# johndpope/Emote-hack

Measured on AMD Instinct MI355X. Metric: denoised frames/s (512x512, 50-step DDPM), higher is better.
Workload: dtype bf16; 1 GPU; cfg2 (BASELINE configs[1]): 512x512 latents 64x64, 12-frame window per GPU, 50-step DDPM, CFG 7.5 (uc+c batched), ReferenceNet on (midup), motion modules res 1/2/4/8, ctx 77x768; 1 step = 1 loop iteration + 1/10 of a 10-timestep ReferenceNet pass; frames_total=12, num_inference_steps=50, latents_finite=True, hip_graphs=True, reference_group=10

## Files before the change

### emote_hack_amd/csrc/temporal.hip

```cpp
#include "common.h"

static constexpr int TA_THREADS = 256;


template <typename T>
__global__ __launch_bounds__(TA_THREADS) void temporal_attention_kernel(const T* __restrict__ qkv, int64_t ldqkv, T* __restrict__ out,
                                                                        int64_t ldo, int F, int HW, int C, int d, int hpb, int P,
                                                                        float scale, int JW, int FP) {
  constexpr int V = TT<T>::VEC;
  extern __shared__ __attribute__((aligned(16))) unsigned char smem[];
  const int CT = hpb * d;
  const int ROW = P * CT * (int)sizeof(T) + 16;
  unsigned char* Qs = smem;
  unsigned char* Ks = Qs + F * ROW;
  unsigned char* Vs = Ks + F * ROW;
  float* S = (float*)(Vs + F * ROW);

  const int tid = threadIdx.x;
  const int pix0 = blockIdx.x * P, hg = blockIdx.y, b = blockIdx.z;
  const int c0 = hg * CT;
  const int CTV = CT / V, PC = P * CTV;
  const int jl = tid % JW, rstep = TA_THREADS / JW, r0 = tid / JW;

  for (int j0 = 0; j0 < PC; j0 += JW) {
    const int j = j0 + jl;
    if (j >= PC || r0 >= rstep) break;
    const int pp = j / CTV, cv = j - pp * CTV;
    const bool pix_ok = pix0 + pp < HW;
    const T* src = qkv + ((int64_t)(b * F + r0) * HW + (pix_ok ? pix0 + pp : 0)) * ldqkv + c0 + cv * V;
    const int64_t fstep = (int64_t)rstep * HW * ldqkv;
    unsigned char* dst = smem + j * 16;
#pragma unroll 4
    for (int f = r0; f < F; f += rstep) {
      uint4 vq = make_uint4(0, 0, 0, 0), vk = vq, vv = vq;
      if (pix_ok) { vq = *(const uint4*)src; vk = *(const uint4*)(src + C); vv = *(const uint4*)(src + 2 * C); }
      *(uint4*)(dst + f * ROW) = vq;
      *(uint4*)(dst + (F + f) * ROW) = vk;
      *(uint4*)(dst + (2 * F + f) * ROW) = vv;
      src += fstep;
    }
  }
  __syncthreads();

  const int dv = d / V, NPH = P * hpb;
  {
    const int nb = (F + 2) / 3, per = nb * nb;
    for (int it = tid; it < NPH * per; it += TA_THREADS) {
      const int ph = it / per, r = it - ph * per, bq = r / nb, bk = r - bq * nb;
      const unsigned char* qp[3];
      const unsigned char* kp[3];
#pragma unroll
      for (int u = 0; u < 3; u++) {
        const int fq = bq * 3 + u < F ? bq * 3 + u : F - 1, fk = bk * 3 + u < F ? bk * 3 + u : F - 1;
        qp[u] = Qs + fq * ROW + ph * d * (int)sizeof(T);
        kp[u] = Ks + fk * ROW + ph * d * (int)sizeof(T);
      }
      float acc[3][3] = {{0.f, 0.f, 0.f}, {0.f, 0.f, 0.f}, {0.f, 0.f, 0.f}};
      for (int c = 0; c < dv; c++) {
        uint4 qv[3], kv[3];
#pragma unroll
        for (int u = 0; u < 3; u++) { qv[u] = *(const uint4*)(qp[u] + c * 16); kv[u] = *(const uint4*)(kp[u] + c * 16); }
#pragma unroll
        for (int u = 0; u < 3; u++)
#pragma unroll
          for (int w = 0; w < 3; w++) acc[u][w] = dot16<T>(qv[u], kv[w], acc[u][w]);
      }
      float* sp = S + ph * F * F;
#pragma unroll
      for (int u = 0; u < 3; u++)
#pragma unroll
        for (int w = 0; w < 3; w++) {
          const int fq = bq * 3 + u, fk = bk * 3 + w;
          if (fq < F && fk < F) sp[fq * F + fk] = acc[u][w] * scale;
        }
    }
  }
  __syncthreads();

  for (int i = tid; i < NPH * F; i += TA_THREADS) {
    float* row = S + i * F;
    float mx = -1e30f;
    for (int k = 0; k < F; k++) mx = fmaxf(mx, row[k]);
    float sum = 0.f;
    for (int k = 0; k < F; k++) { float e = __expf(row[k] - mx); row[k] = e; sum += e; }
    const float inv = 1.0f / sum;
    for (int k = 0; k < F; k++) {
      float w = row[k] * inv;
      w = round_through<T>(w);
      row[k] = w;
    }
  }
  __syncthreads();

  for (int j0 = 0; j0 < PC; j0 += JW) {
    const int j = j0 + jl;
    if (j >= PC || r0 >= rstep) break;
    const int pp = j / CTV, cv = j - pp * CTV;
    if (pix0 + pp >= HW) continue;
    const int hh = (cv * V) / d;
    const float* pbase = S + (pp * hpb + hh) * F * F;
    const unsigned char* vp = Vs + j * 16;
    for (int fq0 = r0; fq0 < F; fq0 += 4 * rstep) {
      float acc[4][V];
#pragma unroll
      for (int u = 0; u < 4; u++)
#pragma unroll
        for (int e = 0; e < V; e++) acc[u][e] = 0.f;
      for (int fk = 0; fk < F; fk++) {
        float vv[V];
        unpack16<T>(*(const uint4*)(vp + fk * ROW), vv);
#pragma unroll
        for (int u = 0; u < 4; u++) {
          const int fq = fq0 + u * rstep;
          const float w = fq < F ? pbase[fq * F + fk] : 0.f;
#pragma unroll
          for (int e = 0; e < V; e++) acc[u][e] += w * vv[e];
        }
      }
#pragma unroll
      for (int u = 0; u < 4; u++) {
        const int fq = fq0 + u * rstep;
        if (fq < F) *(uint4*)(out + ((int64_t)(b * F + fq) * HW + pix0 + pp) * ldo + c0 + cv * V) = pack16<T>(acc[u]);
      }
    }
  }
}

typedef __bf16 ta_bf16x8 __attribute__((ext_vector_type(8)));
typedef _Float16 ta_f16x8 __attribute__((ext_vector_type(8)));
typedef short ta_s16x4 __attribute__((ext_vector_type(4)));
typedef _Float16 ta_f16x4 __attribute__((ext_vector_type(4)));
template <typename T> __device__ __forceinline__ f32x4 ta_mma32(const uint4& a, const uint4& b, f32x4 c);
template <> __device__ __forceinline__ f32x4 ta_mma32<bf16_t>(const uint4& a, const uint4& b, f32x4 c) {
  return __builtin_amdgcn_mfma_f32_16x16x32_bf16(__builtin_bit_cast(ta_bf16x8, a), __builtin_bit_cast(ta_bf16x8, b), c, 0, 0, 0);
}
template <> __device__ __forceinline__ f32x4 ta_mma32<f16_t>(const uint4& a, const uint4& b, f32x4 c) {
  return __builtin_amdgcn_mfma_f32_16x16x32_f16(__builtin_bit_cast(ta_f16x8, a), __builtin_bit_cast(ta_f16x8, b), c, 0, 0, 0);
}
template <typename T> __device__ __forceinline__ f32x4 ta_mma16(const uint2& a, const uint2& b, f32x4 c);
template <> __device__ __forceinline__ f32x4 ta_mma16<bf16_t>(const uint2& a, const uint2& b, f32x4 c) {
  return __builtin_amdgcn_mfma_f32_16x16x16bf16_1k(__builtin_bit_cast(ta_s16x4, a), __builtin_bit_cast(ta_s16x4, b), c, 0, 0, 0);
}
template <> __device__ __forceinline__ f32x4 ta_mma16<f16_t>(const uint2& a, const uint2& b, f32x4 c) {
  return __builtin_amdgcn_mfma_f32_16x16x16f16(__builtin_bit_cast(ta_f16x4, a), __builtin_bit_cast(ta_f16x4, b), c, 0, 0, 0);
}
template <typename OP> __device__ __forceinline__ float ta_allreduce_groups(float x, OP op) {
  auto a = __builtin_amdgcn_permlane16_swap(__float_as_uint(x), __float_as_uint(x), false, false);
  const float y = op(__uint_as_float(a[0]), __uint_as_float(a[1]));
  auto b = __builtin_amdgcn_permlane32_swap(__float_as_uint(y), __float_as_uint(y), false, false);
  return op(__uint_as_float(b[0]), __uint_as_float(b[1]));
}

static constexpr int TAM_WAVES = 4;
template <typename T, int NFB>
__global__ __launch_bounds__(64 * TAM_WAVES) void temporal_attention_mfma_kernel(const T* __restrict__ qkv, int64_t ldqkv, T* __restrict__ out,
                                                                                 int64_t ldo, int F, int HW, int C, int d, int heads,
                                                                                 float c_exp, int64_t items, int wave_lds) {
  static_assert(sizeof(T) == 2, "MFMA temporal attention: 2-byte element types");
  extern __shared__ __attribute__((aligned(16))) unsigned char smem[];
  const int lane = threadIdx.x & 63, wave = __builtin_amdgcn_readfirstlane(threadIdx.x >> 6);
  const int fr = lane & 15, g = lane >> 4;
  const int dch = d / 8, vrow = d * 2;
  unsigned char* vimg = smem + wave * wave_lds;
  const unsigned vimg_a = (unsigned)(uintptr_t)(__attribute__((address_space(3))) unsigned char*)vimg;
  for (int off = F * vrow + lane * 16; off < wave_lds; off += 64 * 16) *(uint4*)(vimg + off) = make_uint4(0, 0, 0, 0);
  bool f_ok[NFB];
#pragma unroll
  for (int fb = 0; fb < NFB; fb++) f_ok[fb] = fb * 16 + fr < F;
  const int nvec = F * dch;
  const int ksteps = (d + 31) / 32, nblocks = (d + 15) / 16;
  const unsigned tr_lane = vimg_a + (4 * g + (fr >> 2)) * vrow + (fr & 3) * 8;
  for (int64_t item = (int64_t)blockIdx.x * TAM_WAVES + wave; item < items; item += (int64_t)gridDim.x * TAM_WAVES) {
    const int head = (int)(item % heads);
    const int64_t bp = item / heads;
    const int pix = (int)(bp % HW), b = (int)(bp / HW);
    const int64_t row0 = (int64_t)b * F * HW + pix;
    const T* base = qkv + head * d;
    for (int j0 = 0; j0 < nvec; j0 += 64) {
      const int j = j0 + lane;
      if (j < nvec) {
        const int fk = j / dch, c = j - fk * dch;
        __builtin_amdgcn_global_load_lds((const __attribute__((address_space(1))) void*)(base + (row0 + (int64_t)fk * HW) * ldqkv + 2 * C + c * 8),
                                         (__attribute__((address_space(3))) void*)(vimg + j0 * 16), 16, 0, 0);
      }
    }
    const T* qrow[NFB];
#pragma unroll
    for (int fb = 0; fb < NFB; fb++) qrow[fb] = base + (row0 + (int64_t)(f_ok[fb] ? fb * 16 + fr : 0) * HW) * ldqkv;
    f32x4 s[NFB][NFB];
#pragma unroll
    for (int kb = 0; kb < NFB; kb++)
#pragma unroll
      for (int qb = 0; qb < NFB; qb++) s[kb][qb] = f32x4{0.f, 0.f, 0.f, 0.f};
    for (int ks = 0; ks < ksteps; ks++) {
      const int c = ks * 4 + g;
      uint4 kf[NFB], qf[NFB];
#pragma unroll
      for (int fb = 0; fb < NFB; fb++) {
        kf[fb] = make_uint4(0, 0, 0, 0); qf[fb] = kf[fb];
        if (f_ok[fb] && c < dch) { qf[fb] = *(const uint4*)(qrow[fb] + c * 8); kf[fb] = *(const uint4*)(qrow[fb] + C + c * 8); }
      }
#pragma unroll
      for (int kb = 0; kb < NFB; kb++)
#pragma unroll
        for (int qb = 0; qb < NFB; qb++) s[kb][qb] = ta_mma32<T>(kf[kb], qf[qb], s[kb][qb]);
    }
    uint2 pb[NFB][NFB];
#pragma unroll
    for (int qb = 0; qb < NFB; qb++) {
      float p[NFB][4];
      float mx = -1e30f;
#pragma unroll
      for (int kb = 0; kb < NFB; kb++)
#pragma unroll
        for (int r = 0; r < 4; r++) { p[kb][r] = (kb * 16 + 4 * g + r < F) ? s[kb][qb][r] : -1e30f; mx = fmaxf(mx, p[kb][r]); }
      mx = ta_allreduce_groups(mx, [](float x, float y) { return fmaxf(x, y); });
      float sum = 0.f;
#pragma unroll
      for (int kb = 0; kb < NFB; kb++)
#pragma unroll
        for (int r = 0; r < 4; r++) { p[kb][r] = __builtin_amdgcn_exp2f((p[kb][r] - mx) * c_exp); sum += p[kb][r]; }
      sum = ta_allreduce_groups(sum, [](float x, float y) { return x + y; });
      const float inv = 1.0f / sum;
#pragma unroll
      for (int kb = 0; kb < NFB; kb++) pb[kb][qb] = make_uint2(pack2<T>(p[kb][0] * inv, p[kb][1] * inv), pack2<T>(p[kb][2] * inv, p[kb][3] * inv));
    }
    asm volatile("s_waitcnt vmcnt(0)" ::: "memory");
    T* orow[NFB];
#pragma unroll
    for (int qb = 0; qb < NFB; qb++) orow[qb] = out + (row0 + (int64_t)(f_ok[qb] ? qb * 16 + fr : 0) * HW) * ldo + head * d + 4 * g;
    for (int nb = 0; nb < nblocks; nb++) {
      uint2 vf[NFB];
#pragma unroll
      for (int kb = 0; kb < NFB; kb++)
        asm volatile("ds_read_b64_tr_b16 %0, %1" : "=&v"(vf[kb]) : "v"(tr_lane + kb * 16 * vrow + nb * 32) : "memory");
      asm volatile("s_waitcnt lgkmcnt(0)" ::: "memory");
      __builtin_amdgcn_sched_barrier(0);
#pragma unroll
      for (int qb = 0; qb < NFB; qb++) {
        f32x4 o = {0.f, 0.f, 0.f, 0.f};
#pragma unroll
        for (int kb = 0; kb < NFB; kb++) o = ta_mma16<T>(vf[kb], pb[kb][qb], o);
        if (f_ok[qb] && nb * 16 + 4 * g < d) *(uint2*)(orow[qb] + nb * 16) = make_uint2(pack2<T>(o[0], o[1]), pack2<T>(o[2], o[3]));
      }
    }
  }
}

template <typename T>
static void launch_temporal_mfma(const void* qkv, int64_t ldqkv, void* out, int64_t ldo, int B, int F, int HW, int heads, int d, float scale,
                                 hipStream_t st) {
  const int nfb = F <= 16 ? 1 : 2, C = heads * d;
  const int64_t items = (int64_t)B * HW * heads;
  const int wave_lds = 16 * nfb * d * 2 + 64;
  int64_t gx = (items + TAM_WAVES - 1) / TAM_WAVES;
  if (gx > 256 * 8) gx = 256 * 8;
  const float c_exp = scale * 1.4426950408889634f;
  if (nfb == 1)
    temporal_attention_mfma_kernel<T, 1><<<(unsigned)gx, 64 * TAM_WAVES, TAM_WAVES * wave_lds, st>>>((const T*)qkv, ldqkv, (T*)out, ldo, F, HW, C, d, heads, c_exp,
                                                                                                       items, wave_lds);
  else
    temporal_attention_mfma_kernel<T, 2><<<(unsigned)gx, 64 * TAM_WAVES, TAM_WAVES * wave_lds, st>>>((const T*)qkv, ldqkv, (T*)out, ldo, F, HW, C, d, heads, c_exp,
                                                                                                       items, wave_lds);
}

extern "C" int emo_temporal_attention(const void* qkv, int64_t ldqkv, void* out, int64_t ldo, int B, int F, int HW, int heads, int d,
                                      float scale, int dtype, void* stream) {
  EMO_CHECK(qkv && out, EMO_ERR_NULL, "emo_temporal_attention: null pointer");
  EMO_CHECK(emo_dtype_ok(dtype), EMO_ERR_BAD_DTYPE, "emo_temporal_attention: dtype %d", dtype);
  const int V = emo_dtype_vec(dtype), esz = dtype == EMO_F32 ? 4 : 2;
  EMO_CHECK(B > 0 && F > 0 && F <= 32 && HW > 0 && heads > 0 && d > 0, EMO_ERR_BAD_SHAPE, "emo_temporal_attention: B=%d F=%d HW=%d", B, F, HW);
  EMO_CHECK(d % V == 0 && ldqkv % V == 0 && ldo % V == 0, EMO_ERR_BAD_SHAPE, "emo_temporal_attention: d=%d must be a multiple of %d", d, V);
  const int C = heads * d;
  EMO_CHECK(ldqkv >= 3 * C && ldo >= C, EMO_ERR_BAD_SHAPE, "emo_temporal_attention: leading dims");
  if (dtype != EMO_F32 && d % 8 == 0 && d <= 256 && TAM_WAVES * (16 * (F <= 16 ? 1 : 2) * d * 2 + 64) <= 64 * 1024) {
    if (dtype == EMO_BF16) launch_temporal_mfma<bf16_t>(qkv, ldqkv, out, ldo, B, F, HW, heads, d, scale, as_stream(stream));
    else launch_temporal_mfma<f16_t>(qkv, ldqkv, out, ldo, B, F, HW, heads, d, scale, as_stream(stream));
    EMO_LAUNCH_CHECK();
    return EMO_OK;
  }
  const int budget = 48 * 1024, lds_plain = 64 * 1024, lds_max = 160 * 1024;
  auto need = [&](int h, int pp) { return (size_t)3 * F * ((size_t)pp * h * d * esz + 16) + (size_t)pp * h * F * F * 4; };
  int hpb = heads;
  while (hpb > 1 && (hpb % 2 == 0) && need(hpb, 1) > (size_t)budget) hpb /= 2;
  if (hpb > 1 && need(hpb, 1) > (size_t)lds_plain) {
    do { hpb--; } while (hpb > 1 && (heads % hpb != 0 || need(hpb, 1) > (size_t)budget));
  }
  int P = 1;
  while (P < 8 && P * 2 <= HW && need(hpb, 2 * P) <= (size_t)budget) P *= 2;
  const size_t lds = need(hpb, P);
  EMO_CHECK(lds <= (size_t)lds_max, EMO_ERR_UNSUPPORTED, "emo_temporal_attention: LDS %zu", lds);
  if (lds > (size_t)lds_plain) {
    static bool once[3] = {false, false, false};
    if (!once[dtype]) {
      hipError_t e = hipSuccess;
      EMO_DISPATCH(dtype, "emo_temporal_attention",
                   e = hipFuncSetAttribute((const void*)temporal_attention_kernel<T>, hipFuncAttributeMaxDynamicSharedMemorySize, (int)lds_max));
      if (e != hipSuccess) return emo_fail(EMO_ERR_HIP, "emo_temporal_attention: hipFuncSetAttribute: %s", hipGetErrorString(e));
      once[dtype] = true;
    }
  }
  EMO_CHECK(B <= 65535 && heads / hpb <= 65535, EMO_ERR_BAD_SHAPE, "emo_temporal_attention: grid limits");
  dim3 grid((HW + P - 1) / P, heads / hpb, B);
  const int JW = P * hpb * d / V < TA_THREADS ? P * hpb * d / V : TA_THREADS;
  const int FP = F <= 16 ? 16 : 32;
  hipStream_t st = as_stream(stream);
  EMO_DISPATCH(dtype, "emo_temporal_attention",
               (temporal_attention_kernel<T><<<grid, TA_THREADS, lds, st>>>((const T*)qkv, ldqkv, (T*)out, ldo, F, HW, C, d, hpb, P, scale, JW, FP)));
  EMO_LAUNCH_CHECK();
  return EMO_OK;
}
```

Before: 6.085 frames/s.

## Prefetch next item's Q/K in temporal MFMA attention and stage output through LDS

The MFMA temporal attention kernel now issues the next work item's V-to-LDS copy and Q/K register loads right after finishing the current item, so global latency overlaps with compute. Output tiles are written into the LDS V image and then stored with coalesced 16-byte writes instead of scattered 8-byte stores. The K-step count is now a template parameter so the fragments can stay in registers. The launcher picks 4 or 8 waves per block and sizes the grid from an occupancy query and an LDS budget. In exchange it raises register pressure and adds a one-time occupancy query on the host.

```diff
diff --git a/emote_hack_amd/csrc/temporal.hip b/emote_hack_amd/csrc/temporal.hip
--- a/emote_hack_amd/csrc/temporal.hip
+++ b/emote_hack_amd/csrc/temporal.hip
@@ -151,59 +151,97 @@
   return op(__uint_as_float(b[0]), __uint_as_float(b[1]));
 }
 
-static constexpr int TAM_WAVES = 4;
-template <typename T, int NFB>
-__global__ __launch_bounds__(64 * TAM_WAVES) void temporal_attention_mfma_kernel(const T* __restrict__ qkv, int64_t ldqkv, T* __restrict__ out,
+static constexpr int TAM_WAVES_MIN = 4, TAM_WAVES_MAX = 8;
+static inline int tam_image_bytes(int nfb, int d) { return 16 * nfb * d * 2 + ((d + 15) / 16 * 32 - d * 2); }
+
+template <typename T, int NFB, int KS>
+__global__ __launch_bounds__(64 * TAM_WAVES_MAX) void temporal_attention_mfma_kernel(const T* __restrict__ qkv, int64_t ldqkv, T* __restrict__ out,
                                                                                  int64_t ldo, int F, int HW, int C, int d, int heads,
-                                                                                 float c_exp, int64_t items, int wave_lds) {
+                                                                                 float c_exp, int64_t items, int img_lds) {
   static_assert(sizeof(T) == 2, "MFMA temporal attention: 2-byte element types");
+  constexpr int KR = KS > 0 ? KS : 1;
   extern __shared__ __attribute__((aligned(16))) unsigned char smem[];
   const int lane = threadIdx.x & 63, wave = __builtin_amdgcn_readfirstlane(threadIdx.x >> 6);
   const int fr = lane & 15, g = lane >> 4;
   const int dch = d / 8, vrow = d * 2;
-  unsigned char* vimg = smem + wave * wave_lds;
+  unsigned char* vimg = smem + wave * img_lds;
   const unsigned vimg_a = (unsigned)(uintptr_t)(__attribute__((address_space(3))) unsigned char*)vimg;
-  for (int off = F * vrow + lane * 16; off < wave_lds; off += 64 * 16) *(uint4*)(vimg + off) = make_uint4(0, 0, 0, 0);
+  for (int off = F * vrow + lane * 16; off < img_lds; off += 64 * 16) *(uint4*)(vimg + off) = make_uint4(0, 0, 0, 0);
   bool f_ok[NFB];
 #pragma unroll
   for (int fb = 0; fb < NFB; fb++) f_ok[fb] = fb * 16 + fr < F;
   const int nvec = F * dch;
   const int ksteps = (d + 31) / 32, nblocks = (d + 15) / 16;
   const unsigned tr_lane = vimg_a + (4 * g + (fr >> 2)) * vrow + (fr & 3) * 8;
-  for (int64_t item = (int64_t)blockIdx.x * TAM_WAVES + wave; item < items; item += (int64_t)gridDim.x * TAM_WAVES) {
-    const int head = (int)(item % heads);
-    const int64_t bp = item / heads;
+  const int waves = blockDim.x >> 6;
+  const int64_t stride = (int64_t)gridDim.x * waves;
+  int64_t item = (int64_t)blockIdx.x * waves + wave;
+  if (item >= items) return;
+  uint4 kf[KR][NFB], qf[KR][NFB];
+  int rq_head;
+  int64_t rq_row0;
+  auto request = [&](int64_t it) {
+    rq_head = (int)(it % heads);
+    const int64_t bp = it / heads;
     const int pix = (int)(bp % HW), b = (int)(bp / HW);
-    const int64_t row0 = (int64_t)b * F * HW + pix;
-    const T* base = qkv + head * d;
+    rq_row0 = (int64_t)b * F * HW + pix;
+    const T* base = qkv + rq_head * d;
     for (int j0 = 0; j0 < nvec; j0 += 64) {
       const int j = j0 + lane;
       if (j < nvec) {
         const int fk = j / dch, c = j - fk * dch;
-        __builtin_amdgcn_global_load_lds((const __attribute__((address_space(1))) void*)(base + (row0 + (int64_t)fk * HW) * ldqkv + 2 * C + c * 8),
+        __builtin_amdgcn_global_load_lds((const __attribute__((address_space(1))) void*)(base + (rq_row0 + (int64_t)fk * HW) * ldqkv + 2 * C + c * 8),
                                          (__attribute__((address_space(3))) void*)(vimg + j0 * 16), 16, 0, 0);
       }
     }
-    const T* qrow[NFB];
-#pragma unroll
-    for (int fb = 0; fb < NFB; fb++) qrow[fb] = base + (row0 + (int64_t)(f_ok[fb] ? fb * 16 + fr : 0) * HW) * ldqkv;
+    if constexpr (KS > 0) {
+#pragma unroll
+      for (int fb = 0; fb < NFB; fb++) {
+        const T* qr = base + (rq_row0 + (int64_t)(f_ok[fb] ? fb * 16 + fr : 0) * HW) * ldqkv;
+#pragma unroll
+        for (int ks = 0; ks < KS; ks++) {
+          const int c = ks * 4 + g;
+          kf[ks][fb] = make_uint4(0, 0, 0, 0); qf[ks][fb] = kf[ks][fb];
+          if (f_ok[fb] && c < dch) { qf[ks][fb] = *(const uint4*)(qr + c * 8); kf[ks][fb] = *(const uint4*)(qr + C + c * 8); }
+        }
+      }
+    }
+  };
+  request(item);
+  for (;;) {
+    const int head = rq_head;
+    const int64_t row0 = rq_row0;
+    const int64_t nxt = item + stride;
     f32x4 s[NFB][NFB];
 #pragma unroll
     for (int kb = 0; kb < NFB; kb++)
 #pragma unroll
       for (int qb = 0; qb < NFB; qb++) s[kb][qb] = f32x4{0.f, 0.f, 0.f, 0.f};
-    for (int ks = 0; ks < ksteps; ks++) {
-      const int c = ks * 4 + g;
-      uint4 kf[NFB], qf[NFB];
-#pragma unroll
-      for (int fb = 0; fb < NFB; fb++) {
-        kf[fb] = make_uint4(0, 0, 0, 0); qf[fb] = kf[fb];
-        if (f_ok[fb] && c < dch) { qf[fb] = *(const uint4*)(qrow[fb] + c * 8); kf[fb] = *(const uint4*)(qrow[fb] + C + c * 8); }
-      }
-#pragma unroll
-      for (int kb = 0; kb < NFB; kb++)
-#pragma unroll
-        for (int qb = 0; qb < NFB; qb++) s[kb][qb] = ta_mma32<T>(kf[kb], qf[qb], s[kb][qb]);
+    if constexpr (KS > 0) {
+      asm volatile("s_waitcnt vmcnt(0)" ::: "memory");
+#pragma unroll
+      for (int ks = 0; ks < KS; ks++)
+#pragma unroll
+        for (int kb = 0; kb < NFB; kb++)
+#pragma unroll
+          for (int qb = 0; qb < NFB; qb++) s[kb][qb] = ta_mma32<T>(kf[ks][kb], qf[ks][qb], s[kb][qb]);
+    } else {
+      const T* base = qkv + head * d;
+      const T* qrow[NFB];
+#pragma unroll
+      for (int fb = 0; fb < NFB; fb++) qrow[fb] = base + (row0 + (int64_t)(f_ok[fb] ? fb * 16 + fr : 0) * HW) * ldqkv;
+      for (int ks = 0; ks < ksteps; ks++) {
+        const int c = ks * 4 + g;
+#pragma unroll
+        for (int fb = 0; fb < NFB; fb++) {
+          kf[0][fb] = make_uint4(0, 0, 0, 0); qf[0][fb] = kf[0][fb];
+          if (f_ok[fb] && c < dch) { qf[0][fb] = *(const uint4*)(qrow[fb] + c * 8); kf[0][fb] = *(const uint4*)(qrow[fb] + C + c * 8); }
+        }
+#pragma unroll
+        for (int kb = 0; kb < NFB; kb++)
+#pragma unroll
+          for (int qb = 0; qb < NFB; qb++) s[kb][qb] = ta_mma32<T>(kf[0][kb], qf[0][qb], s[kb][qb]);
+      }
     }
     uint2 pb[NFB][NFB];
 #pragma unroll
@@ -225,10 +263,7 @@
 #pragma unroll
       for (int kb = 0; kb < NFB; kb++) pb[kb][qb] = make_uint2(pack2<T>(p[kb][0] * inv, p[kb][1] * inv), pack2<T>(p[kb][2] * inv, p[kb][3] * inv));
     }
-    asm volatile("s_waitcnt vmcnt(0)" ::: "memory");
-    T* orow[NFB];
-#pragma unroll
-    for (int qb = 0; qb < NFB; qb++) orow[qb] = out + (row0 + (int64_t)(f_ok[qb] ? qb * 16 + fr : 0) * HW) * ldo + head * d + 4 * g;
+    if constexpr (KS == 0) asm volatile("s_waitcnt vmcnt(0)" ::: "memory");
     for (int nb = 0; nb < nblocks; nb++) {
       uint2 vf[NFB];
 #pragma unroll
@@ -241,27 +276,60 @@
         f32x4 o = {0.f, 0.f, 0.f, 0.f};
 #pragma unroll
         for (int kb = 0; kb < NFB; kb++) o = ta_mma16<T>(vf[kb], pb[kb][qb], o);
-        if (f_ok[qb] && nb * 16 + 4 * g < d) *(uint2*)(orow[qb] + nb * 16) = make_uint2(pack2<T>(o[0], o[1]), pack2<T>(o[2], o[3]));
-      }
-    }
-  }
+        if (f_ok[qb] && nb * 16 + 4 * g < d)
+          *(uint2*)(vimg + (qb * 16 + fr) * vrow + (nb * 16 + 4 * g) * 2) = make_uint2(pack2<T>(o[0], o[1]), pack2<T>(o[2], o[3]));
+      }
+    }
+    for (int j0 = 0; j0 < nvec; j0 += 64) {
+      const int j = j0 + lane;
+      if (j < nvec) {
+        const int fq = j / dch, c = j - fq * dch;
+        *(uint4*)(out + (row0 + (int64_t)fq * HW) * ldo + head * d + c * 8) = *(const uint4*)(vimg + j * 16);
+      }
+    }
+    if (nxt >= items) break;
+    request(nxt);
+    item = nxt;
+  }
+}
+
+struct tam_args {
+  const void* qkv; int64_t ldqkv; void* out; int64_t ldo; int F, HW, C, d, heads; float c_exp; int64_t items; int img_lds; hipStream_t st;
+};
+template <typename T, int NFB, int KS>
+static hipError_t launch_temporal_mfma_as(const tam_args& a) {
+  const int big = TAM_WAVES_MAX * a.img_lds <= 64 * 1024, waves = big ? TAM_WAVES_MAX : TAM_WAVES_MIN;
+  static int by_registers[2] = {0, 0};
+  if (!by_registers[big]) {
+    int n = 0;
+    const hipError_t e = hipOccupancyMaxActiveBlocksPerMultiprocessor(&n, temporal_attention_mfma_kernel<T, NFB, KS>, 64 * waves, 0);
+    if (e != hipSuccess) return e;
+    by_registers[big] = n < 1 ? 1 : n < 32 / waves ? n : 32 / waves;
+  }
+  const size_t lds = (size_t)waves * a.img_lds;
+  const int by_lds = (int)(160 * 1024 / ((lds + 1279) / 1280 * 1280));
+  const int64_t cap = (int64_t)256 * (by_lds < by_registers[big] ? by_lds : by_registers[big]) * waves;
+  const int64_t walk = (a.items + cap - 1) / cap;
+  const int64_t gx = (a.items + waves * walk - 1) / (waves * walk);
+  temporal_attention_mfma_kernel<T, NFB, KS><<<(unsigned)gx, 64 * waves, lds, a.st>>>((const T*)a.qkv, a.ldqkv, (T*)a.out, a.ldo, a.F, a.HW, a.C, a.d, a.heads,
+                                                                                     a.c_exp, a.items, a.img_lds);
+  return hipSuccess;
 }
 
 template <typename T>
-static void launch_temporal_mfma(const void* qkv, int64_t ldqkv, void* out, int64_t ldo, int B, int F, int HW, int heads, int d, float scale,
-                                 hipStream_t st) {
-  const int nfb = F <= 16 ? 1 : 2, C = heads * d;
-  const int64_t items = (int64_t)B * HW * heads;
-  const int wave_lds = 16 * nfb * d * 2 + 64;
-  int64_t gx = (items + TAM_WAVES - 1) / TAM_WAVES;
-  if (gx > 256 * 8) gx = 256 * 8;
-  const float c_exp = scale * 1.4426950408889634f;
-  if (nfb == 1)
-    temporal_attention_mfma_kernel<T, 1><<<(unsigned)gx, 64 * TAM_WAVES, TAM_WAVES * wave_lds, st>>>((const T*)qkv, ldqkv, (T*)out, ldo, F, HW, C, d, heads, c_exp,
-                                                                                                       items, wave_lds);
-  else
-    temporal_attention_mfma_kernel<T, 2><<<(unsigned)gx, 64 * TAM_WAVES, TAM_WAVES * wave_lds, st>>>((const T*)qkv, ldqkv, (T*)out, ldo, F, HW, C, d, heads, c_exp,
-                                                                                                       items, wave_lds);
+static hipError_t launch_temporal_mfma(const void* qkv, int64_t ldqkv, void* out, int64_t ldo, int B, int F, int HW, int heads, int d, float scale,
+                                       hipStream_t st) {
+  const int nfb = F <= 16 ? 1 : 2, ks = (d + 31) / 32;
+  const tam_args a = {qkv, ldqkv, out, ldo, F, HW, heads * d, d, heads, scale * 1.4426950408889634f, (int64_t)B * HW * heads, tam_image_bytes(nfb, d), st};
+#define TAM_KS(KS) (nfb == 1 ? launch_temporal_mfma_as<T, 1, KS>(a) : launch_temporal_mfma_as<T, 2, KS>(a))
+  switch (ks) {
+    case 1: return TAM_KS(1);
+    case 2: return TAM_KS(2);
+    case 3: return TAM_KS(3);
+    case 5: return TAM_KS(5);
+    default: return TAM_KS(0);
+  }
+#undef TAM_KS
 }
 
 extern "C" int emo_temporal_attention(const void* qkv, int64_t ldqkv, void* out, int64_t ldo, int B, int F, int HW, int heads, int d,
@@ -273,9 +341,10 @@
   EMO_CHECK(d % V == 0 && ldqkv % V == 0 && ldo % V == 0, EMO_ERR_BAD_SHAPE, "emo_temporal_attention: d=%d must be a multiple of %d", d, V);
   const int C = heads * d;
   EMO_CHECK(ldqkv >= 3 * C && ldo >= C, EMO_ERR_BAD_SHAPE, "emo_temporal_attention: leading dims");
-  if (dtype != EMO_F32 && d % 8 == 0 && d <= 256 && TAM_WAVES * (16 * (F <= 16 ? 1 : 2) * d * 2 + 64) <= 64 * 1024) {
-    if (dtype == EMO_BF16) launch_temporal_mfma<bf16_t>(qkv, ldqkv, out, ldo, B, F, HW, heads, d, scale, as_stream(stream));
-    else launch_temporal_mfma<f16_t>(qkv, ldqkv, out, ldo, B, F, HW, heads, d, scale, as_stream(stream));
+  if (dtype != EMO_F32 && d % 8 == 0 && d <= 256 && TAM_WAVES_MIN * (16 * (F <= 16 ? 1 : 2) * d * 2 + 64) <= 64 * 1024) {
+    const hipError_t e = dtype == EMO_BF16 ? launch_temporal_mfma<bf16_t>(qkv, ldqkv, out, ldo, B, F, HW, heads, d, scale, as_stream(stream))
+                                           : launch_temporal_mfma<f16_t>(qkv, ldqkv, out, ldo, B, F, HW, heads, d, scale, as_stream(stream));
+    if (e != hipSuccess) return emo_fail(EMO_ERR_HIP, "emo_temporal_attention: occupancy query: %s", hipGetErrorString(e));
     EMO_LAUNCH_CHECK();
     return EMO_OK;
   }
```

Measured after the change: 6.117 frames/s, median of 6. Within noise of the previous version (+0.5%).
